# avik-pal/LocalRegNeuralDE.jl

Measured on AMD Instinct MI355X. Metric: NFE/s (vector-field evals/s inside the adaptive Tsit5 NeuralODE forward, MNIST-ODE B=512/GPU), higher is better.
Workload: dtype f32; 1 GPU; MNIST-ODE MLP field TDChain(Dense(785=>100,tanh),Dense(101=>784)), B=512/GPU, Tsit5 adaptive abstol=reltol=1.4e-08, tspan=(0,1), regularize=unbiased/error_estimate, forward pass (solve + local reg step); global_batch=512, parallelism=batch-shard x1

## Files before the change

localregneuralde.jl_amd/csrc/lrnde_kernels.hip:

```cpp
#include <hip/hip_runtime.h>
#include <rccl/rccl.h>

#include <math.h>
#include <stdarg.h>
#include <stddef.h>
#include <stdio.h>
#include <stdlib.h>
#include <string.h>

#include <algorithm>
#include <type_traits>
#include <chrono>
#include <mutex>
#include <string>
#include <functional>
#include <vector>

#include "lrnde.h"
#include "lrnde_hooks.h"
#include "lrnde_math.hpp"
#include "lrnde_comm.hpp"

namespace {

// ... 814 lines not shown
}

constexpr int PROG_RING = 32;
template <class A> __device__ __forceinline__ void solve_progress(const A& a, int j, const CtrlHead& c, int nsaved_done, float steps_left) {
  if (!a.prog) return;
  if (c.status != ST_RUNNING) *reinterpret_cast<CtrlHead*>(a.fin_host) = c;
  const unsigned long long cnt = (unsigned long long)(j + 1) & 0xffffffull;
  const unsigned long long stt = (unsigned long long)(c.status & 0xff);
  const unsigned long long nsv = (unsigned long long)(nsaved_done > 65535 ? 65535 : nsaved_done);
  const float sl = __builtin_ceilf(steps_left);
  const unsigned long long rem = (unsigned long long)(sl > 65535.f ? 65535 : (sl > 0.f ? (int)sl : 0));
  __hip_atomic_store(a.prog + (j & (PROG_RING - 1)), cnt | (stt << 24) | (nsv << 32) | (rem << 48), __ATOMIC_RELAXED, __HIP_MEMORY_SCOPE_SYSTEM);
}

template <class T> __device__ __forceinline__ T pin_v(T x) { asm volatile("" : "+v"(x)); return x; }
struct PrologueArgs {
  int mode, maxiters, nsave, cap_saved, save_everystep, exact_pow, nwg_global, dense_cap, dense_direct, force_store_k, cap_trace;
  float t0, t1;
  double n_global;
  Ctrl* ctrl; const double* part_recv; const double* pinit_recv; const float* saveat; float* dense; lrnde_trace_row* trace;
  unsigned long long* prog; Ctrl* fin_host;
};
__device__ __forceinline__ PrologueArgs pin_args(const StepArgs& a) {
  PrologueArgs p{};
  p.mode = pin_v(a.mode); p.maxiters = pin_v(a.maxiters); p.nsave = pin_v(a.nsave); p.cap_saved = pin_v(a.cap_saved);
  p.save_everystep = pin_v(a.save_everystep); p.exact_pow = pin_v(a.exact_pow); p.nwg_global = pin_v(a.nwg_global);
  p.dense_cap = pin_v(a.dense_cap); p.dense_direct = pin_v(a.dense_direct); p.force_store_k = pin_v(a.force_store_k);
  p.cap_trace = pin_v(a.cap_trace); p.t0 = pin_v(a.t0); p.t1 = pin_v(a.t1); p.n_global = pin_v(a.n_global);
  p.ctrl = pin_v(a.ctrl); p.part_recv = pin_v(a.part_recv); p.pinit_recv = pin_v(a.pinit_recv); p.saveat = pin_v(a.saveat);
  p.dense = pin_v(a.dense); p.trace = pin_v(a.trace); p.prog = pin_v(a.prog); p.fin_host = pin_v(a.fin_host);
  return p;
}

__device__ __forceinline__ void step_prologue(const StepArgs& a_, int j, Bcast* bc) {
  const int lane = threadIdx.x & 63;
  if (a_.mode == MODE_BENCH) {
    if (lane == 0) { bc->do_step = 1; bc->cur = 0; bc->t = a_.t0; bc->dt = a_.bench_dt; bc->accepted_prev = 0; bc->store_k = 0; bc->dense_idx = -1; bc->dense_slot = -1; bc->isave0 = 0; bc->isave1 = 0; }
    return;
  }
  const PrologueArgs a = pin_args(a_);
  PSTAMP(0);
  const CtrlHead* cin = reinterpret_cast<const CtrlHead*>(a.ctrl + (j & 1));
  CtrlHead c = *cin;
  CtrlHead* cout = reinterpret_cast<CtrlHead*>(a.ctrl + ((j + 1) & 1));
  const double* ppart = a.part_recv + (size_t)(j & 1) * a.nwg_global * PSTRIDE;
  PartLoads pl;
  part_issue<false>(pl, ppart, a.nwg_global);
  float svl = 0.f;
  if (lane < a.nsave) svl = a.saveat[lane];
  auto saveat_at = [&](int is) -> float {
    return is < 64 ? __shfl(svl, is, 64) : a.saveat[is];
  };
  if (c.status != ST_RUNNING) {
    if (blockIdx.x == 0 && lane == 0) { *cout = c; solve_progress(a, j, c, c.nsaved, 0.f); }
    if (lane == 0) bc->do_step = 0, bc->accepted_prev = 0;
    return;
  }
  const float gamma = 0.9f, qmin = 0.2f, qmax = 10.0f, qoldinit = 1e-4f;
  const float beta1 = (float)(7.0 / 50.0), beta2 = (float)(2.0 / 25.0);
  const float dtmax = a.t1 - a.t0;
  const float dtmin = fmaxf_(eps_f(a.t1), eps_f(a.t0));
  int accepted = 0, do_step = 0;
  float t = c.t, dt = c.dt;
  Bcast b;
  b.accepted_prev = 0; b.cur_prev = c.cur; b.isave0 = c.isave; b.isave1 = c.isave; b.nsaved0 = c.nsaved;
  b.t_new = c.t; b.tprev = c.t; b.dt_prev = c.dt; b.dt0 = 0.f; b.dense_idx = -1;

  if (c.first) {
    if (a.mode != MODE_SINGLE_GIVEN_DT) {
      const Sum3 r1 = reduce_partials3(a.pinit_recv, a.nwg_global);
      const Sum3 r2 = reduce_partials3(a.pinit_recv + (size_t)a.nwg_global * PSTRIDE, a.nwg_global);
      dt = init_dt_final3(r1, r2, a.n_global, dtmax);
      c.nf = 3;
    }
    c.dt_init = dt;
    c.dtpropose = dt;
  } else {
    PSTAMP(1);
    const float pq = a.exact_pow ? (float)pow((double)c.qold, (double)beta2) : fastpow(c.qold, beta2);
    const float ttmp = c.t + c.dt;
    const float t_acc = (__builtin_fabsf(ttmp - a.t1) < 100.0f * eps_f(fmaxf_(c.t, a.t1))) ? a.t1 : ttmp;
    const float floor_acc = fmaxf_(eps_f(t_acc), dtmin);
// ... 941 lines not shown
  const int nwg = (B + NB - 1) / NB;
  const size_t sm = smem_bytes(c->m.Dp, c->m.Hp);
  if (vecw(c) == 4) {
    if (spec) hipLaunchKernelGGL((k_step<4, true>), dim3(nwg), dim3(NT), sm, c->stream, a, j);
    else hipLaunchKernelGGL((k_step<4, false>), dim3(nwg), dim3(NT), sm, c->stream, a, j);
  } else {
    if (spec) hipLaunchKernelGGL((k_step<1, true>), dim3(nwg), dim3(NT), sm, c->stream, a, j);
    else hipLaunchKernelGGL((k_step<1, false>), dim3(nwg), dim3(NT), sm, c->stream, a, j);
  }
  HIPCHK(c, hipGetLastError());
  return LRNDE_OK;
}

int exchange(lrnde_ctx* c, double* send, double* recv, size_t count) {
  if (!sharded(c)) return LRNDE_OK;
  return comm_allreduce(c, send, recv, count, true);
}

int run_init(lrnde_ctx* c, int B, const StepArgs& a) {
  int rc;
  const size_t cnt = (size_t)a.nwg_global * PSTRIDE;
  const bool qt = use_qtile(c, B);
  const int nq = (B + QNB - 1) / QNB;
  if (c->field) {
    const int nwg = (B + CNB - 1) / CNB;
    const size_t sm = chain_smem_bytes(c->cd.wfloats);
    hipLaunchKernelGGL(k_init1_chain, dim3(nwg), dim3(NT), sm, c->stream, a, c->cd);
    HIPCHK(c, hipGetLastError());
    if ((rc = exchange(c, c->pinit, c->pinit_rx, cnt))) return rc;
    hipLaunchKernelGGL(k_init2_chain, dim3(nwg), dim3(NT), sm, c->stream, a, c->cd);
    HIPCHK(c, hipGetLastError());
    return exchange(c, c->pinit + cnt, c->pinit_rx + cnt, cnt);
  }
  if (qt) { hipLaunchKernelGGL(k_init1_q, dim3(nq), dim3(QNT), smem_q(c), c->stream, a); rc = LRNDE_OK; HIPCHK(c, hipGetLastError()); }
  else if (vecw(c) == 4) rc = launch_tile_kernel(c, k_init1<4>, B, a);
  else rc = launch_tile_kernel(c, k_init1<1>, B, a);
  if (rc) return rc;
  if ((rc = exchange(c, c->pinit, c->pinit_rx, cnt))) return rc;
  if (qt) { hipLaunchKernelGGL(k_init2_q, dim3(nq), dim3(QNT), smem_q(c), c->stream, a); rc = LRNDE_OK; HIPCHK(c, hipGetLastError()); }
  else if (vecw(c) == 4) rc = launch_tile_kernel(c, k_init2<4>, B, a);
  else rc = launch_tile_kernel(c, k_init2<1>, B, a);
  if (rc) return rc;
  return exchange(c, c->pinit + cnt, c->pinit_rx + cnt, cnt);
}

int set_smem_attr() {
  static bool done = false;
  if (done) return 0;
  const int maxb = 160 * 1024;
  hipFuncSetAttribute((const void*)k_step<4, false>, hipFuncAttributeMaxDynamicSharedMemorySize, maxb);
  hipFuncSetAttribute((const void*)k_step<1, false>, hipFuncAttributeMaxDynamicSharedMemorySize, maxb);
  hipFuncSetAttribute((const void*)k_step<4, true>, hipFuncAttributeMaxDynamicSharedMemorySize, maxb);
  hipFuncSetAttribute((const void*)k_step<1, true>, hipFuncAttributeMaxDynamicSharedMemorySize, maxb);
  hipFuncSetAttribute((const void*)k_init1<4>, hipFuncAttributeMaxDynamicSharedMemorySize, maxb);
  hipFuncSetAttribute((const void*)k_init1<1>, hipFuncAttributeMaxDynamicSharedMemorySize, maxb);
  hipFuncSetAttribute((const void*)k_init2<4>, hipFuncAttributeMaxDynamicSharedMemorySize, maxb);
  hipFuncSetAttribute((const void*)k_init2<1>, hipFuncAttributeMaxDynamicSharedMemorySize, maxb);
  hipFuncSetAttribute((const void*)k_rhs<4>, hipFuncAttributeMaxDynamicSharedMemorySize, maxb);
  hipFuncSetAttribute((const void*)k_rhs<1>, hipFuncAttributeMaxDynamicSharedMemorySize, maxb);
  hipFuncSetAttribute((const void*)k_step_q<false, 1>, hipFuncAttributeMaxDynamicSharedMemorySize, maxb);
  hipFuncSetAttribute((const void*)k_step_q<true, 1>, hipFuncAttributeMaxDynamicSharedMemorySize, maxb);
  hipFuncSetAttribute((const void*)k_step_q<false, 4>, hipFuncAttributeMaxDynamicSharedMemorySize, maxb);
  hipFuncSetAttribute((const void*)k_step_q<true, 4>, hipFuncAttributeMaxDynamicSharedMemorySize, maxb);
  hipFuncSetAttribute((const void*)k_init1_q, hipFuncAttributeMaxDynamicSharedMemorySize, maxb);
  hipFuncSetAttribute((const void*)k_init2_q, hipFuncAttributeMaxDynamicSharedMemorySize, maxb);
  hipFuncSetAttribute((const void*)k_rhs_q, hipFuncAttributeMaxDynamicSharedMemorySize, maxb);
  hipFuncSetAttribute((const void*)k_vjp<4>, hipFuncAttributeMaxDynamicSharedMemorySize, maxb);
  hipFuncSetAttribute((const void*)k_vjp<1>, hipFuncAttributeMaxDynamicSharedMemorySize, maxb);
  hipFuncSetAttribute((const void*)k_sde_step<4>, hipFuncAttributeMaxDynamicSharedMemorySize, maxb);
  hipFuncSetAttribute((const void*)k_sde_step<1>, hipFuncAttributeMaxDynamicSharedMemorySize, maxb);
  hipFuncSetAttribute((const void*)k_sde_rkmil<4>, hipFuncAttributeMaxDynamicSharedMemorySize, maxb);
  hipFuncSetAttribute((const void*)k_sde_rkmil<1>, hipFuncAttributeMaxDynamicSharedMemorySize, maxb);
// ... 2708 lines not shown
```

localregneuralde.jl_amd/csrc/lrnde_qtile.hpp:

```cpp

constexpr int QNB = 4;
constexpr int QNW = 7;
constexpr int QNT = QNW * 64;
constexpr int QB1 = 7;
constexpr int QSEG = 28;
constexpr int QB2 = 4;
constexpr int QRGC = 4;

struct SmemQ {
  f32x4* xl;
  f32x4* hl;
  f32x4* pl;
  float* bias;
  double* red;
  Bcast* bc;
};

__device__ __forceinline__ int q_nseg1(const ModelDev& m) { return (m.KQ1p + QSEG - 1) / QSEG; }
__host__ __device__ __forceinline__ int q_w2_groups(int KQ1p) { return 2 * ((KQ1p + QSEG - 1) / QSEG); }

__device__ __forceinline__ float q_segment_sum(const float* plf, int ne, int e, int nseg) {
  float vals[QNW];
#pragma unroll
  for (int sgi = 0; sgi < QNW; ++sgi) vals[sgi] = plf[(size_t)(sgi < nseg ? sgi : nseg - 1) * ne + e];
  float v = vals[0];
#pragma unroll
  for (int sgi = 1; sgi < QNW; ++sgi) v = sgi < nseg ? v + vals[sgi] : v;
  return v;
}


__device__ __forceinline__ SmemQ carve_q(const ModelDev& m) {
  extern __shared__ __attribute__((aligned(16))) char smem[];
  SmemQ s;
  s.xl = reinterpret_cast<f32x4*>(smem);
  s.hl = s.xl + (size_t)m.KQ1p * 4;
  s.pl = s.hl + (size_t)m.KQ2p * 4;
  s.bias = reinterpret_cast<float*>(s.pl + (size_t)q_nseg1(m) * m.RG1 * 64);
  s.red = reinterpret_cast<double*>(s.bias + 128 * (size_t)(m.RG1 + m.RG2));
  s.bc = reinterpret_cast<Bcast*>(s.red + QNW * 3);
  return s;
}
__device__ __forceinline__ f32x4* q_extra_smem(const SmemQ& s) {
  extern __shared__ __attribute__((aligned(16))) char smem[];
  const unsigned off = (unsigned)(reinterpret_cast<const char*>(s.bc + 1) - smem);
  return reinterpret_cast<f32x4*>(smem + ((off + 15u) & ~15u));
}
static size_t smem_bytes_q(int KQ1p, int KQ2p, int RG1, int RG2) {
  const size_t nseg1 = (size_t)((KQ1p + QSEG - 1) / QSEG);
  return ((size_t)KQ1p * 4 + (size_t)KQ2p * 4 + nseg1 * RG1 * 64) * 16 + 128 * (size_t)(RG1 + RG2) * 4 +
         QNW * 3 * sizeof(double) + sizeof(Bcast) + 16;
}
template <bool SKIP0 = false>
__device__ __forceinline__ void smem_init_q(const ModelDev& m, const SmemQ& s) {
  const f32x4 z = {0.f, 0.f, 0.f, 0.f};
  constexpr int NTH = SKIP0 ? QNT - 64 : QNT;
  const int tid = SKIP0 ? (int)threadIdx.x - 64 : (int)threadIdx.x;
  if (SKIP0 && tid < 0) return;
  for (int i = tid; i < (m.KQ1p + m.KQ2p) * 4; i += NTH) s.xl[i] = z;
  const int h64 = m.RG1 * 64, d64 = m.RG2 * 64;
  for (int i = tid; i < h64; i += NTH) {
    s.bias[i] = (i < m.Hp) ? m.w1t[i] : 0.f;
    s.bias[h64 + i] = (i < m.Hp) ? m.b1[i] : 0.f;
  }
  for (int i = tid; i < d64; i += NTH) {
    s.bias[2 * h64 + i] = (i < m.Dp) ? m.w2t[i] : 0.f;
    s.bias[2 * h64 + d64 + i] = (i < m.Dp) ? m.b2[i] : 0.f;
  }
}

struct TileIOQ {
  __amdgpu_buffer_rsrc_t rs;
  int voff;
};
__device__ __forceinline__ TileIOQ make_tile_io_q(const StepArgs& a, int b0, int nvalid) {
  const int lane = threadIdx.x & 63, sidx = lane & 3, q = lane >> 2;
  TileIOQ io;
  io.rs = __builtin_amdgcn_make_buffer_rsrc((void*)a.state, 0, (int)(a.n_local * 40), 0x00020000);
  io.voff = (sidx < nvalid) ? ((b0 + sidx) * a.m.D + q * 4) * 4 : 0x7ffffff0;
  return io;
}
__device__ __forceinline__ int q_voff(const TileIOQ& io, int rb, bool own) {
  return own ? io.voff + rb * 4 : 0x7ffffff0;
}
__device__ __forceinline__ f32x4 qload(const TileIOQ& io, int voff_rg, int soff) {
  return __builtin_bit_cast(f32x4, __builtin_amdgcn_raw_buffer_load_b128(io.rs, voff_rg, soff, 0));
}
__device__ __forceinline__ void qstore(const TileIOQ& io, int voff_rg, int soff, const f32x4& v) {
  __builtin_amdgcn_raw_buffer_store_b128(__builtin_bit_cast(u32x4, v), io.rs, voff_rg + soff, 0, 0);
}

struct EpiStoreKQ {
  static constexpr int NPRE = 1;
  const ModelDev* m; float* kout; int b0, nvalid;
  __device__ __forceinline__ void pre(int, bool, f32x4 (&)[NPRE]) const {}
  __device__ __forceinline__ void post(int rb, bool own, const f32x4& kv, f32x4 (&)[NPRE]) const {
    const int lane = threadIdx.x & 63, sidx = lane & 3, q = lane >> 2;
    const int row0 = rb + q * 4;
    if (sidx < nvalid && own) *reinterpret_cast<f32x4*>(kout + (size_t)(b0 + sidx) * m->D + row0) = kv;
  }
};

template <int S> struct EpiStageQ {
  static constexpr int NPRE = S;
  TileIOQ io;
  int off_up, off_k[6], off_out, off_x;
  float dt;
  f32x4* xl;
  f32x4* kl; int KL;
  const f32x4* klu; const f32x4* klk;
  int store_k;
  __device__ __forceinline__ void pre(int rb, bool, f32x4 (&pb)[NPRE]) const {
    const int li = rb + (threadIdx.x & 63);
    pb[0] = klu[li];
    if (S > 1) pb[S > 1 ? 1 : 0] = klk[li];
#pragma unroll
    for (int j = 2; j < S; ++j) pb[j] = kl[(size_t)(j + 2) * KL + li];
  }
  __device__ __forceinline__ void post(int rb, bool own, const f32x4& kv, f32x4 (&pb)[NPRE]) const {
    const int lane = threadIdx.x & 63, sidx = lane & 3, q = lane >> 2;
    constexpr int off = (S - 1) * S / 2;
    const int vo = q_voff(io, rb, own);
    qstore(io, store_k ? vo : 0x7ffffff0, off_out, kv);
    if (own) kl[(size_t)(S + 2) * KL + rb + lane] = kv;
    f32x4 x;
#pragma unroll
    for (int r = 0; r < 4; ++r) {
      float o[S];
#pragma unroll
      for (int j = 0; j < S - 1; ++j) o[j] = pb[1 + j][r];
      o[S - 1] = kv[r];
      float sum = (float)Tsit5::A[off] * o[0] + (float)Tsit5::A[off + 1] * o[1];
// ... 272 lines not shown
          acc0 = qmfma(st.ring[SL][j][0].x, b_[j].x, acc0);
          acc1 = qmfma(st.ring[SL][j][1].x, b_[j].x, acc1);
          acc0 = qmfma(st.ring[SL][j][0].y, b_[j].y, acc0);
          acc1 = qmfma(st.ring[SL][j][1].y, b_[j].y, acc1);
          acc0 = qmfma(st.ring[SL][j][0].z, b_[j].z, acc0);
          acc1 = qmfma(st.ring[SL][j][1].z, b_[j].z, acc1);
          acc0 = qmfma(st.ring[SL][j][0].w, b_[j].w, acc0);
          acc1 = qmfma(st.ring[SL][j][1].w, b_[j].w, acc1);
        }
        LRNDE_QPIN();
      });
      __builtin_amdgcn_sched_barrier(0);
    });
    auto finish = [&](int rb, bool own, const f32x4& tot) {
      const int row0 = own ? rb + q * 4 : 0;
      const f32x4 wt = *reinterpret_cast<const f32x4*>(w2t + row0);
      const f32x4 bb = *reinterpret_cast<const f32x4*>(b2 + row0);
      f32x4 kv;
#pragma unroll
      for (int r = 0; r < 4; ++r) {
        const float pre = m.td ? fma_(wt[r], ts, tot[r]) : tot[r];
        kv[r] = pre + bb[r];
      }
      return kv;
    };
    if (g0 < m.D) epi.post(g0, own0, finish(g0, own0, acc0), pb0);
    if (g1 < m.D) epi.post(g1, own1, finish(g1, own1, acc1), pb1);
  }
  STAMP(5); STAMPW(4);
  __builtin_amdgcn_fence(__ATOMIC_ACQ_REL, "wavefront");
  STAMP(6);
}

template <class F>
__device__ __forceinline__ void q_tile_foreach(const ModelDev& m, int b0, int nvalid, int KQ1, F&& fn) {
  for (int i = threadIdx.x; i < KQ1 * 4; i += QNT) {
    const int sidx = i & 3, kq = i >> 2;
    fn(kq, sidx, sidx < nvalid, (size_t)(b0 + sidx) * m.D + kq * 4);
  }
}

__device__ __forceinline__ f32x4 ld4(const float* p) { return *reinterpret_cast<const f32x4*>(p); }
__device__ __forceinline__ void st4(float* p, const f32x4& v) { *reinterpret_cast<f32x4*>(p) = v; }

__device__ __forceinline__ void block_sum3_q(double* red, double& a, double& b, double& c, bool three = true) {
  const int lane = threadIdx.x & 63;
  const int wave = __builtin_amdgcn_readfirstlane(threadIdx.x >> 6);
  a = wave_sum_dpp(a);
  if (three) { b = wave_sum_dpp(b); c = wave_sum_dpp(c); }
  if (lane == 0) { red[wave * 3 + 0] = a; red[wave * 3 + 1] = b; red[wave * 3 + 2] = c; }
  __syncthreads();
  if (threadIdx.x == 0) {
    double sa = 0.0, sb = 0.0, sc = 0.0;
    for (int w = 0; w < QNW; ++w) { sa += red[w * 3]; sb += red[w * 3 + 1]; sc += red[w * 3 + 2]; }
    a = sa; b = sb; c = sc;
  }
}

__device__ __forceinline__ void q_feval_store(const ModelDev& m, const SmemQ& sm, StreamQ& fc, float ts,
                                              float* kout, int b0, int nvalid) {
  EpiStoreKQ e;
  e.m = &m; e.kout = kout; e.b0 = b0; e.nvalid = nvalid;
  feval_qs<EpiStoreKQ, 0>(m, sm, fc, ts, e);
  __syncthreads();
}

__global__ __launch_bounds__(QNT) void k_rhs_q(StepArgs a, const float* u, float t, float* du) {
  STAMP(0);
  const SmemQ s = carve_q(a.m);
  smem_init_q(a.m, s);
  StreamQ fc;
  stream_init_q(a.m, fc);
  const int b0 = blockIdx.x * QNB, nvalid = min(QNB, a.B - b0);
  const int KQ1 = a.m.D / 4;
  __syncthreads();
  q_tile_foreach(a.m, b0, nvalid, KQ1, [&](int kq, int sidx, bool valid, size_t g) {
    const f32x4 z = {0.f, 0.f, 0.f, 0.f};
    s.xl[kq * 4 + sidx] = valid ? ld4(u + g) : z;
  });
  __syncthreads();
  q_feval_store(a.m, s, fc, t, du, b0, nvalid);
}

__global__ __launch_bounds__(QNT) void k_init1_q(StepArgs a) {
  const SmemQ s = carve_q(a.m);
  smem_init_q(a.m, s);
  StreamQ fc;
  stream_init_q(a.m, fc);
  const int b0 = blockIdx.x * QNB, nvalid = min(QNB, a.B - b0);
  const int KQ1 = a.m.D / 4;
  int cur0; float tinit;
  if (a.init_fresh) {
    cur0 = 0; tinit = a.t0;
    if (blockIdx.x == 0 && threadIdx.x == 0) solve_init_body(a.ctrl, a.t0, a.init_nsaved, a.init_si);
  } else {
    const Ctrl c = a.ctrl[0];
    cur0 = c.cur; tinit = c.t;
  }
  const float* u0 = a.init_u0 ? a.init_u0 : ubuf_at(a, cur0);
  float* ucopy = a.init_u0 ? ubuf_at(a, cur0) : nullptr;
  float* f0 = kfsal_at(a, cur0);
  __syncthreads();
  q_tile_foreach(a.m, b0, nvalid, KQ1, [&](int kq, int sidx, bool valid, size_t g) {
    const f32x4 z = {0.f, 0.f, 0.f, 0.f};
    const f32x4 v = valid ? ld4(u0 + g) : z;
    s.xl[kq * 4 + sidx] = v;
    if (valid && ucopy) st4(ucopy + g, v);
  });
  __syncthreads();
  q_feval_store(a.m, s, fc, tinit, f0, b0, nvalid);
  double a0 = 0.0, a1 = 0.0, a2 = 0.0;
  q_tile_foreach(a.m, b0, nvalid, KQ1, [&](int, int, bool valid, size_t g) {
    if (!valid) return;
    const f32x4 u = ld4(u0 + g), f = ld4(f0 + g);
#pragma unroll
    for (int h = 0; h < 4; ++h) {
      const float sk = a.abstol + __builtin_fabsf(u[h]) * a.reltol;
      const float r0 = u[h] / sk, r1 = f[h] / sk;
      const float q0 = r0 * r0, q1 = r1 * r1;
      a0 += (double)q0; a1 += (double)q1;
    }
  });
  block_sum3_q(s.red, a0, a1, a2);
  publish_partial(a, 2, a0, a1, 0.0);
}

__global__ __launch_bounds__(QNT) void k_init2_q(StepArgs a) {
  const SmemQ s = carve_q(a.m);
  smem_init_q(a.m, s);
  StreamQ fc;
  stream_init_q(a.m, fc);
  const int b0 = blockIdx.x * QNB, nvalid = min(QNB, a.B - b0);
  const int KQ1 = a.m.D / 4;
  const Ctrl c = a.ctrl[0];
  if (threadIdx.x < 64) {
    double s1[3];
    reduce_partials(a.pinit_recv, a.nwg_global, s1);
    if (threadIdx.x == 0) s.bc->dt0 = init_dt0(s1, a.n_global, a.t1 - a.t0);
  }
  __syncthreads();
  const float dt0 = s.bc->dt0;
  const float* u0 = ubuf_at(a, c.cur);
  const float* f0 = kfsal_at(a, c.cur);
  float* f1 = a.ks[0];
  q_tile_foreach(a.m, b0, nvalid, KQ1, [&](int kq, int sidx, bool valid, size_t g) {
    f32x4 x = {0.f, 0.f, 0.f, 0.f};
    if (valid) {
      const f32x4 u = ld4(u0 + g), f = ld4(f0 + g);
#pragma unroll
      for (int h = 0; h < 4; ++h) x[h] = u[h] + dt0 * f[h];
    }
    s.xl[kq * 4 + sidx] = x;
  });
  __syncthreads();
  q_feval_store(a.m, s, fc, c.t + dt0, f1, b0, nvalid);
  double a0 = 0.0, a1 = 0.0, a2 = 0.0;
  q_tile_foreach(a.m, b0, nvalid, KQ1, [&](int, int, bool valid, size_t g) {
    if (!valid) return;
    const f32x4 u = ld4(u0 + g), f = ld4(f0 + g), ff = ld4(f1 + g);
#pragma unroll
    for (int h = 0; h < 4; ++h) {
      const float sk = a.abstol + __builtin_fabsf(u[h]) * a.reltol;
      const float r2 = (ff[h] - f[h]) / sk;
      const float q2 = r2 * r2;
      a0 += (double)q2;
    }
  });
  block_sum3_q(s.red, a0, a1, a2);
  publish_partial(a, 3, a0, 0.0, 0.0);
}

#ifdef LRNDE_DBG_RELOAD
__device__ int g_dbg_bad[8] = {0, 0, 1 << 30, 0, 0, 0, 0, 0};
#endif
template <bool SPEC, int KT> __global__ __launch_bounds__(QNT) void k_step_q(StepArgs a, int j) {
  STAMP(9);
  const SmemQ s = carve_q(a.m);
  StreamQ fc;
  stream_init_q(a.m, fc);
  const int b0 = blockIdx.x * QNB, nvalid = min(QNB, a.B - b0);
  const int KQ1 = a.m.D / 4;
  STAMP(10);
  f32x4* kl = q_extra_smem(s);
  const int KL = a.m.KQ1p * 4;
  if (threadIdx.x < 64) {
    step_prologue(a, j, s.bc);
  } else {
    smem_init_q<true>(a.m, s);
#ifndef LRNDE_NO_PRELOAD
    constexpr int NTH = QNT - 64;
    const int tid = (int)threadIdx.x - 64;
    const f32x4 z = {0.f, 0.f, 0.f, 0.f};
    f32x4 v[3][4];
#pragma unroll
    for (int r = 0; r < 3; ++r) {
      const int i = tid + r * NTH;
      const int sidx = i & 3, kq = i >> 2;
      const bool ok = i < KQ1 * 4 && sidx < nvalid;
      const size_t g = ok ? (size_t)(b0 + sidx) * a.m.D + kq * 4 : 0;
      v[r][0] = ld4(a.ubuf[0] + g); v[r][1] = ld4(a.kfsal[0] + g);
      v[r][2] = ld4(a.ubuf[1] + g); v[r][3] = ld4(a.kfsal[1] + g);
      if (!ok) { v[r][0] = z; v[r][1] = z; v[r][2] = z; v[r][3] = z; }
    }
#pragma unroll
    for (int r = 0; r < 3; ++r) {
      const int i = tid + r * NTH;
      if (i < KQ1 * 4) { kl[i] = v[r][0]; kl[KL + i] = v[r][1]; kl[2 * KL + i] = v[r][2]; kl[3 * KL + i] = v[r][3]; }
    }
#endif
  }
  __syncthreads();
  STAMP(11);
  const Bcast bc = *s.bc;

  if (bc.accepted_prev) {
    const float* up = ubuf_at(a, bc.cur_prev);
    const float* un = ubuf_at(a, bc.cur_prev ^ 1);
    const float* k1 = kfsal_at(a, bc.cur_prev);
    const float* k7 = kfsal_at(a, bc.cur_prev ^ 1);
    int slot = bc.nsaved0;
    for (int is = bc.isave0; is < bc.isave1; ++is, ++slot) {
      const float ts = a.saveat[is];
      float* dst = a.u_saved + (size_t)slot * a.B * a.m.D;
      float* dst2 = slot == a.also_slot ? a.also_dst : nullptr;
      if (ts != bc.t_new) {
        const float theta = (ts - bc.tprev) / bc.dt_prev;
        float bw[7];
        tsit5_bweights(theta, bw);
        q_tile_foreach(a.m, b0, nvalid, KQ1, [&](int, int, bool valid, size_t g) {
          if (!valid) return;
          const f32x4 y0 = ld4(up + g), v1 = ld4(k1 + g), v2 = ld4(a.ks[0] + g), v3 = ld4(a.ks[1] + g),
                      v4 = ld4(a.ks[2] + g), v5 = ld4(a.ks[3] + g), v6 = ld4(a.ks[4] + g), v7 = ld4(k7 + g);
          f32x4 o;
#pragma unroll
          for (int h = 0; h < 4; ++h) {
            float sum = v1[h] * bw[0] + v2[h] * bw[1];
            sum = sum + v3[h] * bw[2];
            sum = sum + v4[h] * bw[3];
            sum = sum + v5[h] * bw[4];
            sum = sum + v6[h] * bw[5];
            sum = sum + v7[h] * bw[6];
            o[h] = y0[h] + bc.dt_prev * sum;
          }
          st4(dst + g, o);
// ... 20 lines not shown
      const size_t nst = (size_t)a.n_local;
      float* dd = a.dense + (size_t)bc.dense_idx * REC_ARRAYS * nst;
      const float* src[8] = {up, k1, a.ks[0], a.ks[1], a.ks[2], a.ks[3], a.ks[4], k7};
      if (!a.dense_direct)
      q_tile_foreach(a.m, b0, nvalid, KQ1, [&](int, int, bool valid, size_t g) {
        if (!valid) return;
        f32x4 v[8], P2, P3, P4;
#pragma unroll
        for (int qq = 0; qq < 8; ++qq) v[qq] = ld4(src[qq] + g);
#pragma unroll
        for (int r = 0; r < 4; ++r) {
          const float kk[6] = {v[2][r], v[3][r], v[4][r], v[5][r], v[6][r], v[7][r]};
          float P[3];
          tsit5_rec_poly(v[1][r], kk, P);
          P2[r] = P[0]; P3[r] = P[1]; P4[r] = P[2];
        }
        st4(dd + g, v[0]); st4(dd + nst + g, v[1]); st4(dd + 2 * nst + g, P2); st4(dd + 3 * nst + g, P3); st4(dd + 4 * nst + g, P4);
      });
      if (blockIdx.x == 0 && threadIdx.x == 0) { a.dense_t[bc.dense_idx] = bc.tprev; a.dense_dt[bc.dense_idx] = bc.dt_prev; }
    }
  }
  if (!bc.do_step) return;

  const float t = bc.t, dt = bc.dt;
  const float c1 = (float)Tsit5::C[0], c2 = (float)Tsit5::C[1], c3 = (float)Tsit5::C[2],
              c4 = (float)Tsit5::C[3];
  double aerr = 0.0, anum = 0.0, aden = 0.0;
  const TileIOQ io = make_tile_io_q(a, b0, nvalid);
  const f32x4* klu = kl + (bc.cur ? 2 : 0) * KL;
  const f32x4* klk = kl + (bc.cur ? 3 : 1) * KL;
  const int o_up = arr_off(a, bc.cur), o_un = arr_off(a, bc.cur ^ 1);
  const int o_k1 = arr_off(a, 2 + bc.cur), o_k7 = arr_off(a, 2 + (bc.cur ^ 1));
  const int o_g6 = arr_off(a, 9);
  __syncthreads();
  {
    const float a21dt = dt * (float)Tsit5::A[0];
    q_tile_foreach(a.m, b0, nvalid, KQ1, [&](int kq, int sidx, bool valid, size_t g) {
#ifdef LRNDE_DBG_RELOAD
      {
        const f32x4 z = {0.f, 0.f, 0.f, 0.f};
        const f32x4 ug = valid ? ld4(ubuf_at(a, bc.cur) + g) : z, fg = valid ? ld4(kfsal_at(a, bc.cur) + g) : z;
        const f32x4 ul = klu[kq * 4 + sidx], fl = klk[kq * 4 + sidx];
        bool bad = false;
        for (int h = 0; h < 4; ++h) bad = bad || __builtin_bit_cast(unsigned, ug[h]) != __builtin_bit_cast(unsigned, ul[h]) || __builtin_bit_cast(unsigned, fg[h]) != __builtin_bit_cast(unsigned, fl[h]);
        if (bad) { atomicAdd(&g_dbg_bad[0], 1); atomicMax(&g_dbg_bad[1], kq * 4 + sidx); atomicMin(&g_dbg_bad[2], kq * 4 + sidx); atomicAdd(&g_dbg_bad[3 + (bc.cur & 1)], 1); }
      }
#endif
#ifdef LRNDE_NO_PRELOAD
      {
        const f32x4 z = {0.f, 0.f, 0.f, 0.f};
        const_cast<f32x4*>(klu)[kq * 4 + sidx] = valid ? ld4(ubuf_at(a, bc.cur) + g) : z;
        const_cast<f32x4*>(klk)[kq * 4 + sidx] = valid ? ld4(kfsal_at(a, bc.cur) + g) : z;
      }
#endif
      const f32x4 u = klu[kq * 4 + sidx], f = klk[kq * 4 + sidx];
      f32x4 x;
#pragma unroll
      for (int h = 0; h < 4; ++h) x[h] = u[h] + a21dt * f[h];
      s.xl[kq * 4 + sidx] = x;
    });
  }
  __syncthreads();
  STAMP(12);
#define LRNDE_QSTAGE(S, TS)                                                             \
  do {                                                                                  \
    EpiStageQ<S> e;                                                                     \
    e.io = io; e.off_up = o_up; e.off_k[0] = o_k1;                                      \
    _Pragma("unroll") for (int qq = 0; qq < 5; ++qq) e.off_k[1 + qq] = arr_off(a, 4 + qq); \
    e.off_out = arr_off(a, 4 + (S - 2));                                                \
    e.off_x = (S == 6) ? o_un : ((S == 5 && a.want_stiff) ? o_g6 : -1);                 \
    e.dt = dt; e.xl = s.xl; e.kl = kl; e.KL = KL; e.klu = klu; e.klk = klk; e.store_k = bc.store_k;  \
    feval_qs<EpiStageQ<S>, (QSB * (S - 2)) % QRING, KT>(a.m, s, fc, (TS), e);                 \
    STAMP(11 + S);                                                                      \
  } while (0)
  LRNDE_QSTAGE(2, t + c1 * dt);
  LRNDE_QSTAGE(3, t + c2 * dt);
  LRNDE_QSTAGE(4, t + c3 * dt);
  LRNDE_QSTAGE(5, t + c4 * dt);
  LRNDE_QSTAGE(6, t + dt);
#undef LRNDE_QSTAGE
  EpiFinalQ ef;
  ef.io = io; ef.off_up = o_up; ef.off_u = o_un; ef.off_k[0] = o_k1;
#pragma unroll
  for (int qq = 0; qq < 5; ++qq) ef.off_k[1 + qq] = arr_off(a, 4 + qq);
  ef.off_g6 = o_g6; ef.off_out = o_k7;
  ef.dt = dt; ef.abstol = a.abstol; ef.reltol = a.reltol; ef.want_stiff = a.want_stiff; ef.nvalid = nvalid;
  ef.D = a.m.D;
  ef.aerr = &aerr; ef.anum = &anum; ef.aden = &aden;
  ef.xl = s.xl; ef.kl = kl; ef.KL = KL; ef.klu = klu; ef.klk = klk;
  ef.rec = a.dense != nullptr && a.dense_direct && bc.dense_slot >= 0; ef.nstB = (int)(a.n_local * 4);
  ef.rsD = __builtin_amdgcn_make_buffer_rsrc((void*)(a.dense + (size_t)(ef.rec ? bc.dense_slot : 0) * REC_ARRAYS * (size_t)a.n_local), 0,
                                             (int)(a.n_local * 4 * REC_ARRAYS), 0x00020000);
  feval_qs<EpiFinalQ, (QSB * 5) % QRING, KT>(a.m, s, fc, t + dt, ef);
  STAMP(18);
  block_sum3_q(s.red, aerr, anum, aden, a.want_stiff != 0);
  STAMP(19);
  publish_partial(a, (j + 1) & 1, aerr, anum, aden);
}

struct BiasPreQ { float w1, b1, w2[2], b2[2]; };
__device__ __forceinline__ BiasPreQ bias_issue_q(const ModelDev& m) {
  BiasPreQ p;
  const int t = (int)threadIdx.x;
  p.w1 = (t < m.Hp) ? m.w1t[t] : 0.f;
  p.b1 = (t < m.Hp) ? m.b1[t] : 0.f;
#pragma unroll
  for (int r = 0; r < 2; ++r) {
    const int i = t + r * QNT;
    p.w2[r] = (i < m.Dp) ? m.w2t[i] : 0.f;
    p.b2[r] = (i < m.Dp) ? m.b2[i] : 0.f;
  }
  return p;
}
__device__ __forceinline__ void smem_zero_q(const ModelDev& m, const SmemQ& s) {
  const f32x4 z = {0.f, 0.f, 0.f, 0.f};
  for (int i = (int)threadIdx.x; i < (m.KQ1p + m.KQ2p) * 4; i += QNT) s.xl[i] = z;
}
__device__ __forceinline__ void bias_write_q(const ModelDev& m, const SmemQ& s, const BiasPreQ& p) {
  const int t = (int)threadIdx.x;
  const int h64 = m.RG1 * 64, d64 = m.RG2 * 64;
  if (t < h64) { s.bias[t] = p.w1; s.bias[h64 + t] = p.b1; }
#pragma unroll
  for (int r = 0; r < 2; ++r) {
    const int i = t + r * QNT;
    if (i < d64) { s.bias[2 * h64 + i] = p.w2[r]; s.bias[2 * h64 + d64 + i] = p.b2[r]; }
  }
}

__global__ void k_pack_q(const float* p, int D, int H, int td, int KQ1p, int KQ2p, int RG1, int G2,
                         float* W1q, float* W2q) {
  const size_t n1 = (size_t)RG1 * KQ1p * 256, n2 = (size_t)G2 * KQ2p * 256;
  const size_t base2 = (size_t)H * (D + td) + H;
  for (size_t i = blockIdx.x * (size_t)blockDim.x + threadIdx.x; i < n1 + n2; i += (size_t)gridDim.x * blockDim.x) {
    if (i < n1) {
      const int jj = i & 3, l = (i >> 2) & 63;
      const size_t blk = i >> 8;
      const int kq = blk % KQ1p, rg = blk / KQ1p;
      const int o = rg * 64 + l, k = kq * 4 + jj;
      W1q[i] = (o < H && k < D) ? p[(size_t)o + (size_t)H * k] : 0.f;
    } else {
      const size_t e = i - n1;
      const int jj = e & 3, l = (e >> 2) & 63;
      const size_t blk = e >> 8;
      const int kq = blk % KQ2p, g = blk / KQ2p;
      const int c = g & 1, o = (g >> 1) * (QSEG * 4) + c * 64 + l, k = kq * 4 + jj;
      const bool mine = c == 0 || l < QSEG * 4 - 64;
      W2q[e] = (mine && o < D && k < H) ? p[base2 + (size_t)o + (size_t)D * k] : 0.f;
    }
  }
}
```

Before: 132,000 NFE/s.

## Partition step-kernel stage-1 input work by segment-owning wave and drop block barrier

In the q-tile step kernel, the preload of u/k buffers and the first-stage input build are now split by wave according to the W1 segment each wave owns. This lets the post-prologue __syncthreads be replaced by a wavefront-scope fence. Bias loads and stream init are issued early, with wave 0 starting them after the prologue's global loads via a callback. The init kernels keep u/f in registers and capture the field output in shared memory instead of re-reading global memory. The intent is to cut block-wide barriers and redundant global loads on the per-step critical path, at the risk of subtle ownership and race bugs if wave-to-segment coverage is wrong.

```diff
diff --git a/localregneuralde.jl_amd/csrc/lrnde_kernels.hip b/localregneuralde.jl_amd/csrc/lrnde_kernels.hip
--- a/localregneuralde.jl_amd/csrc/lrnde_kernels.hip
+++ b/localregneuralde.jl_amd/csrc/lrnde_kernels.hip
@@ -870,10 +870,13 @@
   return p;
 }
 
-__device__ __forceinline__ void step_prologue(const StepArgs& a_, int j, Bcast* bc) {
+struct NoIssue { __device__ void operator()() const {} };
+template <class Issue = NoIssue>
+__device__ __forceinline__ void step_prologue(const StepArgs& a_, int j, Bcast* bc, const Issue& issued = Issue{}) {
   const int lane = threadIdx.x & 63;
   if (a_.mode == MODE_BENCH) {
     if (lane == 0) { bc->do_step = 1; bc->cur = 0; bc->t = a_.t0; bc->dt = a_.bench_dt; bc->accepted_prev = 0; bc->store_k = 0; bc->dense_idx = -1; bc->dense_slot = -1; bc->isave0 = 0; bc->isave1 = 0; }
+    issued();
     return;
   }
   const PrologueArgs a = pin_args(a_);
@@ -886,6 +889,7 @@
   part_issue<false>(pl, ppart, a.nwg_global);
   float svl = 0.f;
   if (lane < a.nsave) svl = a.saveat[lane];
+  issued();
   auto saveat_at = [&](int is) -> float {
     return is < 64 ? __shfl(svl, is, 64) : a.saveat[is];
   };
@@ -1893,12 +1897,13 @@
     HIPCHK(c, hipGetLastError());
     return exchange(c, c->pinit + cnt, c->pinit_rx + cnt, cnt);
   }
-  if (qt) { hipLaunchKernelGGL(k_init1_q, dim3(nq), dim3(QNT), smem_q(c), c->stream, a); rc = LRNDE_OK; HIPCHK(c, hipGetLastError()); }
+  const size_t smqi = smem_q(c) + (size_t)c->m.KQ1p * 4 * 16;
+  if (qt) { hipLaunchKernelGGL(k_init1_q, dim3(nq), dim3(QNT), smqi, c->stream, a); rc = LRNDE_OK; HIPCHK(c, hipGetLastError()); }
   else if (vecw(c) == 4) rc = launch_tile_kernel(c, k_init1<4>, B, a);
   else rc = launch_tile_kernel(c, k_init1<1>, B, a);
   if (rc) return rc;
   if ((rc = exchange(c, c->pinit, c->pinit_rx, cnt))) return rc;
-  if (qt) { hipLaunchKernelGGL(k_init2_q, dim3(nq), dim3(QNT), smem_q(c), c->stream, a); rc = LRNDE_OK; HIPCHK(c, hipGetLastError()); }
+  if (qt) { hipLaunchKernelGGL(k_init2_q, dim3(nq), dim3(QNT), smqi, c->stream, a); rc = LRNDE_OK; HIPCHK(c, hipGetLastError()); }
   else if (vecw(c) == 4) rc = launch_tile_kernel(c, k_init2<4>, B, a);
   else rc = launch_tile_kernel(c, k_init2<1>, B, a);
   if (rc) return rc;
diff --git a/localregneuralde.jl_amd/csrc/lrnde_qtile.hpp b/localregneuralde.jl_amd/csrc/lrnde_qtile.hpp
--- a/localregneuralde.jl_amd/csrc/lrnde_qtile.hpp
+++ b/localregneuralde.jl_amd/csrc/lrnde_qtile.hpp
@@ -51,19 +51,16 @@
   return ((size_t)KQ1p * 4 + (size_t)KQ2p * 4 + nseg1 * RG1 * 64) * 16 + 128 * (size_t)(RG1 + RG2) * 4 +
          QNW * 3 * sizeof(double) + sizeof(Bcast) + 16;
 }
-template <bool SKIP0 = false>
 __device__ __forceinline__ void smem_init_q(const ModelDev& m, const SmemQ& s) {
   const f32x4 z = {0.f, 0.f, 0.f, 0.f};
-  constexpr int NTH = SKIP0 ? QNT - 64 : QNT;
-  const int tid = SKIP0 ? (int)threadIdx.x - 64 : (int)threadIdx.x;
-  if (SKIP0 && tid < 0) return;
-  for (int i = tid; i < (m.KQ1p + m.KQ2p) * 4; i += NTH) s.xl[i] = z;
+  const int tid = (int)threadIdx.x;
+  for (int i = tid; i < (m.KQ1p + m.KQ2p) * 4; i += QNT) s.xl[i] = z;
   const int h64 = m.RG1 * 64, d64 = m.RG2 * 64;
-  for (int i = tid; i < h64; i += NTH) {
+  for (int i = tid; i < h64; i += QNT) {
     s.bias[i] = (i < m.Hp) ? m.w1t[i] : 0.f;
     s.bias[h64 + i] = (i < m.Hp) ? m.b1[i] : 0.f;
   }
-  for (int i = tid; i < d64; i += NTH) {
+  for (int i = tid; i < d64; i += QNT) {
     s.bias[2 * h64 + i] = (i < m.Dp) ? m.w2t[i] : 0.f;
     s.bias[2 * h64 + d64 + i] = (i < m.Dp) ? m.b2[i] : 0.f;
   }
@@ -93,11 +90,13 @@
 struct EpiStoreKQ {
   static constexpr int NPRE = 1;
   const ModelDev* m; float* kout; int b0, nvalid;
+  f32x4* kq;
   __device__ __forceinline__ void pre(int, bool, f32x4 (&)[NPRE]) const {}
   __device__ __forceinline__ void post(int rb, bool own, const f32x4& kv, f32x4 (&)[NPRE]) const {
     const int lane = threadIdx.x & 63, sidx = lane & 3, q = lane >> 2;
     const int row0 = rb + q * 4;
     if (sidx < nvalid && own) *reinterpret_cast<f32x4*>(kout + (size_t)(b0 + sidx) * m->D + row0) = kv;
+    if (kq && own) kq[(rb / 4 + q) * 4 + sidx] = kv;
   }
 };
 
@@ -436,6 +435,35 @@
   STAMP(6);
 }
 
+struct BiasPreQ { float w1, b1, w2[2], b2[2]; };
+__device__ __forceinline__ BiasPreQ bias_issue_q(const ModelDev& m) {
+  BiasPreQ p;
+  const int t = (int)threadIdx.x;
+  p.w1 = (t < m.Hp) ? m.w1t[t] : 0.f;
+  p.b1 = (t < m.Hp) ? m.b1[t] : 0.f;
+#pragma unroll
+  for (int r = 0; r < 2; ++r) {
+    const int i = t + r * QNT;
+    p.w2[r] = (i < m.Dp) ? m.w2t[i] : 0.f;
+    p.b2[r] = (i < m.Dp) ? m.b2[i] : 0.f;
+  }
+  return p;
+}
+__device__ __forceinline__ void smem_zero_q(const ModelDev& m, const SmemQ& s) {
+  const f32x4 z = {0.f, 0.f, 0.f, 0.f};
+  for (int i = (int)threadIdx.x; i < (m.KQ1p + m.KQ2p) * 4; i += QNT) s.xl[i] = z;
+}
+__device__ __forceinline__ void bias_write_q(const ModelDev& m, const SmemQ& s, const BiasPreQ& p) {
+  const int t = (int)threadIdx.x;
+  const int h64 = m.RG1 * 64, d64 = m.RG2 * 64;
+  if (t < h64) { s.bias[t] = p.w1; s.bias[h64 + t] = p.b1; }
+#pragma unroll
+  for (int r = 0; r < 2; ++r) {
+    const int i = t + r * QNT;
+    if (i < d64) { s.bias[2 * h64 + i] = p.w2[r]; s.bias[2 * h64 + d64 + i] = p.b2[r]; }
+  }
+}
+
 template <class F>
 __device__ __forceinline__ void q_tile_foreach(const ModelDev& m, int b0, int nvalid, int KQ1, F&& fn) {
   for (int i = threadIdx.x; i < KQ1 * 4; i += QNT) {
@@ -462,9 +490,9 @@
 }
 
 __device__ __forceinline__ void q_feval_store(const ModelDev& m, const SmemQ& sm, StreamQ& fc, float ts,
-                                              float* kout, int b0, int nvalid) {
+                                              float* kout, int b0, int nvalid, f32x4* kq = nullptr) {
   EpiStoreKQ e;
-  e.m = &m; e.kout = kout; e.b0 = b0; e.nvalid = nvalid;
+  e.m = &m; e.kout = kout; e.b0 = b0; e.nvalid = nvalid; e.kq = kq;
   feval_qs<EpiStoreKQ, 0>(m, sm, fc, ts, e);
   __syncthreads();
 }
@@ -486,13 +514,30 @@
   q_feval_store(a.m, s, fc, t, du, b0, nvalid);
 }
 
+struct InitTileQ {
+  bool v[2];
+  size_t g[2];
+};
+__device__ __forceinline__ InitTileQ init_tile_q(int D, int b0, int nvalid) {
+  InitTileQ t;
+#pragma unroll
+  for (int r = 0; r < 2; ++r) {
+    const int i = (int)threadIdx.x + r * QNT, sidx = i & 3, kq = i >> 2;
+    t.v[r] = kq < D / 4 && sidx < nvalid;
+    t.g[r] = t.v[r] ? (size_t)(b0 + sidx) * D + kq * 4 : 0;
+  }
+  return t;
+}
+
 __global__ __launch_bounds__(QNT) void k_init1_q(StepArgs a) {
   const SmemQ s = carve_q(a.m);
-  smem_init_q(a.m, s);
+  const BiasPreQ bpre = bias_issue_q(a.m);
   StreamQ fc;
   stream_init_q(a.m, fc);
+  smem_zero_q(a.m, s);
   const int b0 = blockIdx.x * QNB, nvalid = min(QNB, a.B - b0);
   const int KQ1 = a.m.D / 4;
+  const f32x4 z = {0.f, 0.f, 0.f, 0.f};
   int cur0; float tinit;
   if (a.init_fresh) {
     cur0 = 0; tinit = a.t0;
@@ -504,19 +549,25 @@
   const float* u0 = a.init_u0 ? a.init_u0 : ubuf_at(a, cur0);
   float* ucopy = a.init_u0 ? ubuf_at(a, cur0) : nullptr;
   float* f0 = kfsal_at(a, cur0);
-  __syncthreads();
-  q_tile_foreach(a.m, b0, nvalid, KQ1, [&](int kq, int sidx, bool valid, size_t g) {
-    const f32x4 z = {0.f, 0.f, 0.f, 0.f};
-    const f32x4 v = valid ? ld4(u0 + g) : z;
-    s.xl[kq * 4 + sidx] = v;
-    if (valid && ucopy) st4(ucopy + g, v);
-  });
-  __syncthreads();
-  q_feval_store(a.m, s, fc, tinit, f0, b0, nvalid);
+  const InitTileQ tq = init_tile_q(a.m.D, b0, nvalid);
+  f32x4 uv[2];
+#pragma unroll
+  for (int r = 0; r < 2; ++r) { uv[r] = ld4(u0 + tq.g[r]); if (!tq.v[r]) uv[r] = z; }
+#pragma unroll
+  for (int r = 0; r < 2; ++r) {
+    const int i = (int)threadIdx.x + r * QNT;
+    if (i < KQ1 * 4) s.xl[i] = uv[r];
+    if (tq.v[r] && ucopy) st4(ucopy + tq.g[r], uv[r]);
+  }
+  bias_write_q(a.m, s, bpre);
+  q_barrier();
+  f32x4* fl = q_extra_smem(s);
+  q_feval_store(a.m, s, fc, tinit, f0, b0, nvalid, fl);
   double a0 = 0.0, a1 = 0.0, a2 = 0.0;
-  q_tile_foreach(a.m, b0, nvalid, KQ1, [&](int, int, bool valid, size_t g) {
-    if (!valid) return;
-    const f32x4 u = ld4(u0 + g), f = ld4(f0 + g);
+#pragma unroll
+  for (int r = 0; r < 2; ++r) {
+    if (!tq.v[r]) continue;
+    const f32x4 u = uv[r], f = fl[(int)threadIdx.x + r * QNT];
 #pragma unroll
     for (int h = 0; h < 4; ++h) {
       const float sk = a.abstol + __builtin_fabsf(u[h]) * a.reltol;
@@ -524,44 +575,57 @@
       const float q0 = r0 * r0, q1 = r1 * r1;
       a0 += (double)q0; a1 += (double)q1;
     }
-  });
+  }
   block_sum3_q(s.red, a0, a1, a2);
   publish_partial(a, 2, a0, a1, 0.0);
 }
 
 __global__ __launch_bounds__(QNT) void k_init2_q(StepArgs a) {
   const SmemQ s = carve_q(a.m);
-  smem_init_q(a.m, s);
+  const BiasPreQ bpre = bias_issue_q(a.m);
   StreamQ fc;
   stream_init_q(a.m, fc);
+  smem_zero_q(a.m, s);
   const int b0 = blockIdx.x * QNB, nvalid = min(QNB, a.B - b0);
   const int KQ1 = a.m.D / 4;
+  const f32x4 z = {0.f, 0.f, 0.f, 0.f};
   const Ctrl c = a.ctrl[0];
+  const float* u0 = ubuf_at(a, c.cur);
+  const float* f0 = kfsal_at(a, c.cur);
+  float* f1 = a.ks[0];
+  const InitTileQ tq = init_tile_q(a.m.D, b0, nvalid);
+  f32x4 uv[2], fv[2];
+#pragma unroll
+  for (int r = 0; r < 2; ++r) {
+    uv[r] = ld4(u0 + tq.g[r]); fv[r] = ld4(f0 + tq.g[r]);
+    if (!tq.v[r]) { uv[r] = z; fv[r] = z; }
+  }
   if (threadIdx.x < 64) {
     double s1[3];
     reduce_partials(a.pinit_recv, a.nwg_global, s1);
     if (threadIdx.x == 0) s.bc->dt0 = init_dt0(s1, a.n_global, a.t1 - a.t0);
   }
-  __syncthreads();
+  bias_write_q(a.m, s, bpre);
+  q_barrier();
   const float dt0 = s.bc->dt0;
-  const float* u0 = ubuf_at(a, c.cur);
-  const float* f0 = kfsal_at(a, c.cur);
-  float* f1 = a.ks[0];
-  q_tile_foreach(a.m, b0, nvalid, KQ1, [&](int kq, int sidx, bool valid, size_t g) {
-    f32x4 x = {0.f, 0.f, 0.f, 0.f};
-    if (valid) {
-      const f32x4 u = ld4(u0 + g), f = ld4(f0 + g);
-#pragma unroll
-      for (int h = 0; h < 4; ++h) x[h] = u[h] + dt0 * f[h];
-    }
-    s.xl[kq * 4 + sidx] = x;
-  });
-  __syncthreads();
-  q_feval_store(a.m, s, fc, c.t + dt0, f1, b0, nvalid);
+#pragma unroll
+  for (int r = 0; r < 2; ++r) {
+    const int i = (int)threadIdx.x + r * QNT;
+    f32x4 x = z;
+    if (tq.v[r]) {
+#pragma unroll
+      for (int h = 0; h < 4; ++h) x[h] = uv[r][h] + dt0 * fv[r][h];
+    }
+    if (i < KQ1 * 4) s.xl[i] = x;
+  }
+  q_barrier();
+  f32x4* fl = q_extra_smem(s);
+  q_feval_store(a.m, s, fc, c.t + dt0, f1, b0, nvalid, fl);
   double a0 = 0.0, a1 = 0.0, a2 = 0.0;
-  q_tile_foreach(a.m, b0, nvalid, KQ1, [&](int, int, bool valid, size_t g) {
-    if (!valid) return;
-    const f32x4 u = ld4(u0 + g), f = ld4(f0 + g), ff = ld4(f1 + g);
+#pragma unroll
+  for (int r = 0; r < 2; ++r) {
+    if (!tq.v[r]) continue;
+    const f32x4 u = uv[r], f = fv[r], ff = fl[(int)threadIdx.x + r * QNT];
 #pragma unroll
     for (int h = 0; h < 4; ++h) {
       const float sk = a.abstol + __builtin_fabsf(u[h]) * a.reltol;
@@ -569,7 +633,7 @@
       const float q2 = r2 * r2;
       a0 += (double)q2;
     }
-  });
+  }
   block_sum3_q(s.red, a0, a1, a2);
   publish_partial(a, 3, a0, 0.0, 0.0);
 }
@@ -581,39 +645,68 @@
   STAMP(9);
   const SmemQ s = carve_q(a.m);
   StreamQ fc;
-  stream_init_q(a.m, fc);
+  BiasPreQ bpre;
+  auto start_stream = [&] { stream_init_q(a.m, fc); bpre = bias_issue_q(a.m); };
+  const int wave = __builtin_amdgcn_readfirstlane(threadIdx.x >> 6);
+  if (wave != 0) start_stream();
   const int b0 = blockIdx.x * QNB, nvalid = min(QNB, a.B - b0);
   const int KQ1 = a.m.D / 4;
   STAMP(10);
   f32x4* kl = q_extra_smem(s);
   const int KL = a.m.KQ1p * 4;
-  if (threadIdx.x < 64) {
-    step_prologue(a, j, s.bc);
+  const int lane = threadIdx.x & 63;
+  const int nseg1 = q_nseg1(a.m);
+  const f32x4 z = {0.f, 0.f, 0.f, 0.f};
+  const int i0 = wave * (QSEG * 4) + lane;
+  const bool has2 = lane < QSEG * 4 - 64;
+  auto pair_off = [&](int i, bool& ok) {
+    const int sidx = i & 3, kq = i >> 2;
+    ok = kq < KQ1 && sidx < nvalid;
+    return ok ? (size_t)(b0 + sidx) * a.m.D + kq * 4 : (size_t)0;
+  };
+  if (wave == 0) {
+    step_prologue(a, j, s.bc, start_stream);
   } else {
-    smem_init_q<true>(a.m, s);
+    const int tid = (int)threadIdx.x - 64;
+    if (tid < a.m.KQ2p * 4) s.hl[tid] = z;
 #ifndef LRNDE_NO_PRELOAD
     constexpr int NTH = QNT - 64;
-    const int tid = (int)threadIdx.x - 64;
-    const f32x4 z = {0.f, 0.f, 0.f, 0.f};
-    f32x4 v[3][4];
-#pragma unroll
-    for (int r = 0; r < 3; ++r) {
-      const int i = tid + r * NTH;
-      const int sidx = i & 3, kq = i >> 2;
-      const bool ok = i < KQ1 * 4 && sidx < nvalid;
-      const size_t g = ok ? (size_t)(b0 + sidx) * a.m.D + kq * 4 : 0;
-      v[r][0] = ld4(a.ubuf[0] + g); v[r][1] = ld4(a.kfsal[0] + g);
-      v[r][2] = ld4(a.ubuf[1] + g); v[r][3] = ld4(a.kfsal[1] + g);
-      if (!ok) { v[r][0] = z; v[r][1] = z; v[r][2] = z; v[r][3] = z; }
-    }
-#pragma unroll
-    for (int r = 0; r < 3; ++r) {
-      const int i = tid + r * NTH;
-      if (i < KQ1 * 4) { kl[i] = v[r][0]; kl[KL + i] = v[r][1]; kl[2 * KL + i] = v[r][2]; kl[3 * KL + i] = v[r][3]; }
-    }
-#endif
-  }
-  __syncthreads();
+    static_assert(4 * QSEG * 4 == NTH + 64, "segment 0's pair items: one per lane of waves 1..6, a second in wave 1");
+    const bool own = wave < nseg1;
+    f32x4 v[2][4], w0[2];
+    bool okv[2], okw[2];
+    if (own) {
+#pragma unroll
+      for (int r = 0; r < 2; ++r) {
+        const size_t g = pair_off(i0 + 64 * r, okv[r]);
+        v[r][0] = ld4(a.ubuf[0] + g); v[r][1] = ld4(a.kfsal[0] + g);
+        v[r][2] = ld4(a.ubuf[1] + g); v[r][3] = ld4(a.kfsal[1] + g);
+      }
+    }
+    auto seg0_item = [&](int p, int& idx, bool& ok) {
+      const int arr = p / (QSEG * 4), i = p - arr * (QSEG * 4);
+      idx = arr * KL + i;
+      const float* src = arr == 0 ? a.ubuf[0] : arr == 1 ? a.kfsal[0] : arr == 2 ? a.ubuf[1] : a.kfsal[1];
+      return src + pair_off(i, ok);
+    };
+    int idx0, idx1 = 0;
+    w0[0] = ld4(seg0_item(tid, idx0, okw[0]));
+    if (wave == 1) w0[1] = ld4(seg0_item(tid + NTH, idx1, okw[1]));
+    if (own) {
+#pragma unroll
+      for (int r = 0; r < 2; ++r) {
+        if (r == 0 || has2) {
+          const int i = i0 + 64 * r;
+          kl[i] = okv[r] ? v[r][0] : z; kl[KL + i] = okv[r] ? v[r][1] : z;
+          kl[2 * KL + i] = okv[r] ? v[r][2] : z; kl[3 * KL + i] = okv[r] ? v[r][3] : z;
+        }
+      }
+    }
+    kl[idx0] = okw[0] ? w0[0] : z;
+    if (wave == 1) kl[idx1] = okw[1] ? w0[1] : z;
+#endif
+  }
+  q_barrier();
   STAMP(11);
   const Bcast bc = *s.bc;
 
@@ -700,35 +793,38 @@
   const int o_up = arr_off(a, bc.cur), o_un = arr_off(a, bc.cur ^ 1);
   const int o_k1 = arr_off(a, 2 + bc.cur), o_k7 = arr_off(a, 2 + (bc.cur ^ 1));
   const int o_g6 = arr_off(a, 9);
-  __syncthreads();
-  {
+  bias_write_q(a.m, s, bpre);
+  if (wave < nseg1) {
     const float a21dt = dt * (float)Tsit5::A[0];
-    q_tile_foreach(a.m, b0, nvalid, KQ1, [&](int kq, int sidx, bool valid, size_t g) {
+#pragma unroll
+    for (int r = 0; r < 2; ++r) {
+      if (r == 1 && !has2) continue;
+      const int i = i0 + 64 * r;
+#if defined(LRNDE_DBG_RELOAD) || defined(LRNDE_NO_PRELOAD)
+      bool valid;
+      const size_t g = pair_off(i, valid);
+#endif
 #ifdef LRNDE_DBG_RELOAD
       {
-        const f32x4 z = {0.f, 0.f, 0.f, 0.f};
         const f32x4 ug = valid ? ld4(ubuf_at(a, bc.cur) + g) : z, fg = valid ? ld4(kfsal_at(a, bc.cur) + g) : z;
-        const f32x4 ul = klu[kq * 4 + sidx], fl = klk[kq * 4 + sidx];
+        const f32x4 ul = klu[i], fl = klk[i];
         bool bad = false;
         for (int h = 0; h < 4; ++h) bad = bad || __builtin_bit_cast(unsigned, ug[h]) != __builtin_bit_cast(unsigned, ul[h]) || __builtin_bit_cast(unsigned, fg[h]) != __builtin_bit_cast(unsigned, fl[h]);
-        if (bad) { atomicAdd(&g_dbg_bad[0], 1); atomicMax(&g_dbg_bad[1], kq * 4 + sidx); atomicMin(&g_dbg_bad[2], kq * 4 + sidx); atomicAdd(&g_dbg_bad[3 + (bc.cur & 1)], 1); }
+        if (bad) { atomicAdd(&g_dbg_bad[0], 1); atomicMax(&g_dbg_bad[1], i); atomicMin(&g_dbg_bad[2], i); atomicAdd(&g_dbg_bad[3 + (bc.cur & 1)], 1); }
       }
 #endif
 #ifdef LRNDE_NO_PRELOAD
-      {
-        const f32x4 z = {0.f, 0.f, 0.f, 0.f};
-        const_cast<f32x4*>(klu)[kq * 4 + sidx] = valid ? ld4(ubuf_at(a, bc.cur) + g) : z;
-        const_cast<f32x4*>(klk)[kq * 4 + sidx] = valid ? ld4(kfsal_at(a, bc.cur) + g) : z;
-      }
-#endif
-      const f32x4 u = klu[kq * 4 + sidx], f = klk[kq * 4 + sidx];
+      const_cast<f32x4*>(klu)[i] = valid ? ld4(ubuf_at(a, bc.cur) + g) : z;
+      const_cast<f32x4*>(klk)[i] = valid ? ld4(kfsal_at(a, bc.cur) + g) : z;
+#endif
+      const f32x4 u = klu[i], f = klk[i];
       f32x4 x;
 #pragma unroll
       for (int h = 0; h < 4; ++h) x[h] = u[h] + a21dt * f[h];
-      s.xl[kq * 4 + sidx] = x;
-    });
-  }
-  __syncthreads();
+      s.xl[i] = x;
+    }
+  }
+  __builtin_amdgcn_fence(__ATOMIC_ACQ_REL, "wavefront");
   STAMP(12);
 #define LRNDE_QSTAGE(S, TS)                                                             \
   do {                                                                                  \
@@ -766,35 +862,6 @@
   publish_partial(a, (j + 1) & 1, aerr, anum, aden);
 }
 
-struct BiasPreQ { float w1, b1, w2[2], b2[2]; };
-__device__ __forceinline__ BiasPreQ bias_issue_q(const ModelDev& m) {
-  BiasPreQ p;
-  const int t = (int)threadIdx.x;
-  p.w1 = (t < m.Hp) ? m.w1t[t] : 0.f;
-  p.b1 = (t < m.Hp) ? m.b1[t] : 0.f;
-#pragma unroll
-  for (int r = 0; r < 2; ++r) {
-    const int i = t + r * QNT;
-    p.w2[r] = (i < m.Dp) ? m.w2t[i] : 0.f;
-    p.b2[r] = (i < m.Dp) ? m.b2[i] : 0.f;
-  }
-  return p;
-}
-__device__ __forceinline__ void smem_zero_q(const ModelDev& m, const SmemQ& s) {
-  const f32x4 z = {0.f, 0.f, 0.f, 0.f};
-  for (int i = (int)threadIdx.x; i < (m.KQ1p + m.KQ2p) * 4; i += QNT) s.xl[i] = z;
-}
-__device__ __forceinline__ void bias_write_q(const ModelDev& m, const SmemQ& s, const BiasPreQ& p) {
-  const int t = (int)threadIdx.x;
-  const int h64 = m.RG1 * 64, d64 = m.RG2 * 64;
-  if (t < h64) { s.bias[t] = p.w1; s.bias[h64 + t] = p.b1; }
-#pragma unroll
-  for (int r = 0; r < 2; ++r) {
-    const int i = t + r * QNT;
-    if (i < d64) { s.bias[2 * h64 + i] = p.w2[r]; s.bias[2 * h64 + d64 + i] = p.b2[r]; }
-  }
-}
-
 __global__ void k_pack_q(const float* p, int D, int H, int td, int KQ1p, int KQ2p, int RG1, int G2,
                          float* W1q, float* W2q) {
   const size_t n1 = (size_t)RG1 * KQ1p * 256, n2 = (size_t)G2 * KQ2p * 256;
```

Result: no change. 133,500 NFE/s (median of 6 runs) (+1.1%).
